# nixorokish/lodestar

Measured on AMD Instinct MI355X. Metric: BLS signature sets verified/sec (1-8 GPUs) + p50 latency @128-set batch, higher is better.
Workload: dtype u32 (381-bit Fp, 12x32-bit Montgomery limbs); 1 GPU; cfg2: 1024 single-pubkey gossip sets per call, batchable requests, random-scalar batch in chunks of 16 requests; each of the 16 contexts submits 22 calls per pass (bls_gpu_verify_many, one device pass, chunks and verdicts per call); sets_per_call=1024, contexts_per_gpu=16, calls_per_pass=22, calls_in_flight_per_gpu=352, parallelism=shard-by-request x1

## Files before the change

__graft_entry__.py:

```python
from __future__ import annotations

import hashlib
import sys
from pathlib import Path

ROOT = Path(__file__).resolve().parent
sys.path.insert(0, str(ROOT))


def build() -> None:
    from lodestar_amd.build import build as build_lib
    from lodestar_amd.build import (build_cpu_baseline, build_deposit_host, build_hostsim, build_napi, build_plan_host,
                                    build_smsum_host)

    build_lib(verbose=True)
    build_napi(verbose=True)
    build_hostsim(verbose=True)
    build_smsum_host(verbose=True)
    build_plan_host(verbose=True)
    build_deposit_host(verbose=True)
    build_cpu_baseline(verbose=True)
    import lodestar_amd
    from lodestar_amd._abi import LIB_PATH

    assert LIB_PATH.exists()


def smoke() -> None:
    from lodestar_amd.native import GpuContext, pack_requests
    from oracle import bls_oracle as O

    with GpuContext(0) as gpu:
        msg = hashlib.sha256(b"lodestar-amd smoke").digest()
        h = gpu.hash_to_g2(msg)[0].tobytes()
        (x0, x1), (y0, y1) = O.hash_to_g2(msg)
        expect = b"".join(v.to_bytes(48, "big") for v in (x1, x0, y1, y0))
        assert h == expect, "hash_to_G2 mismatch against the oracle"

        sks = [O.interop_secret_key(i) for i in range(3)]
        msgs = [hashlib.sha256(b"smoke%d" % i).digest() for i in range(3)]
        sigs = [O.g2_compress(O.sign(s, m)) for s, m in zip(sks, msgs)]
        pks = [O.g1_serialize(O.sk_to_pk(s)) for s in sks]
        sets = list(zip(pks, msgs, sigs))
# ... 10 lines not shown
```

include/lodestar_bls.h:

```cpp
#ifndef LODESTAR_BLS_H
#define LODESTAR_BLS_H

#include <stdint.h>

#ifdef __cplusplus
extern "C" {
#endif

enum {
  BLS_CODE_OK = 0,
  BLS_CODE_BAD_ENCODING = 1,
  BLS_CODE_POINT_NOT_ON_CURVE = 2,
  BLS_CODE_POINT_NOT_IN_GROUP = 3,
  BLS_CODE_PK_IS_INFINITY = 6,
  BLS_CODE_INVALID_SIZE = 8,
  BLS_CODE_ZERO_SIGNATURE = 9,
  BLS_CODE_EMPTY_SET = 10,
  BLS_CODE_EMPTY_AGGREGATE = 11
};

typedef struct bls_batch {
  uint32_t n_sets;
  uint32_t n_reqs;
  const uint32_t* req_set_offsets;
// ... 135 lines not shown
                          uint32_t n_slots, uint32_t* frames_out, uint32_t* flags_out);

int bls_gpu_fpm_bench(bls_gpu_ctx* ctx, uint32_t lanes, uint32_t iters, double* ns_per_fpm, double* fpm_per_s);

int bls_gpu_coop_probe(bls_gpu_ctx* ctx, const char* name, uint32_t blocks, uint32_t reps, double* us_per_step,
                       double* ms_total,
                       uint64_t* step_stamps );

int bls_gpu_kernel_probe(bls_gpu_ctx* ctx, const char* name, uint32_t lanes, uint32_t reps, double* ms);

#define BLS_DEBUG_FORCE_EXACT 1u
#define BLS_DEBUG_NO_MSG_DEDUP 2u
#define BLS_DEBUG_NO_MERGED_CHECK 4u
#define BLS_DEBUG_PACK(n) ((uint32_t)(n) << 8)
#define BLS_DEBUG_PACK_MASK 0x300u
#define BLS_DEBUG_SIGAGG_ON 8u
#define BLS_DEBUG_SIGAGG_OFF 16u
#define BLS_DEBUG_NO_UNITS 32u
#define BLS_DEBUG_MSM 64u
#define BLS_DEBUG_MLF_PL(n) ((uint32_t)(n) << 12)
#define BLS_DEBUG_MLF_PL_MASK 0x7000u
#define BLS_DEBUG_GROUP_TEST 128u
#define BLS_DEBUG_MERGED_EVERY_PASS 0x8000u
int bls_gpu_set_debug_flags(bls_gpu_ctx* ctx, uint32_t flags);

#ifdef __cplusplus
}
#endif

#endif
```

lodestar_amd/_abi.py:

```python
from __future__ import annotations

import ctypes
from pathlib import Path

import os

LIB_PATH = Path(os.environ.get("LODESTAR_BLS_LIB") or Path(__file__).resolve().parent / "_native" / "liblodestar_bls.so")

CODE_OK = 0
CODE_BAD_ENCODING = 1
CODE_POINT_NOT_ON_CURVE = 2
CODE_POINT_NOT_IN_GROUP = 3
CODE_PK_IS_INFINITY = 6
CODE_INVALID_SIZE = 8
CODE_ZERO_SIGNATURE = 9
CODE_EMPTY_SET = 10
CODE_EMPTY_AGGREGATE = 11

ERROR_MESSAGES = {
    CODE_BAD_ENCODING: "BLST_ERROR: BLST_BAD_ENCODING",
    CODE_POINT_NOT_ON_CURVE: "BLST_ERROR: BLST_POINT_NOT_ON_CURVE",
    CODE_POINT_NOT_IN_GROUP: "BLST_ERROR: BLST_POINT_NOT_IN_GROUP",
    CODE_PK_IS_INFINITY: "BLST_ERROR: BLST_PK_IS_INFINITY",
    CODE_INVALID_SIZE: "BLST_ERROR: BLST_INVALID_SIZE",
# ... 39 lines not shown
    "bls_gpu_set_scratch_budget",
    "bls_gpu_request_hw_queues",
)
ERR_ADMISSION = -4
SSZ_ROOT = 0x000 | 32
SSZ_UINT64 = 0x100 | 8
SSZ_CHECKPOINT = 0x200 | 40
SSZ_ATTESTATION_DATA = 0x300 | 128
SSZ_TWO_UINT64 = 0x400 | 16
SSZ_BEACON_BLOCK_HEADER = 0x500 | 112
SSZ_DEPOSIT_MESSAGE = 0x600 | 88
SSZ_FORK_DATA = 0x700 | 36
SSZ_SIGNING_DATA = 0x800 | 64
FIELD_OP_D28 = 0x100
DEBUG_FORCE_EXACT = 1
DEBUG_NO_MSG_DEDUP = 2
DEBUG_NO_MERGED_CHECK = 4
DEBUG_SIGAGG_ON = 8
DEBUG_SIGAGG_OFF = 16
DEBUG_NO_UNITS = 32
DEBUG_MSM = 64
DEBUG_GROUP_TEST = 128
DEBUG_MERGED_EVERY_PASS = 0x8000


def DEBUG_MLF_PL(n: int) -> int:
    return n << 12


def DEBUG_PACK(n: int) -> int:
    return n << 8


class BlsBatch(ctypes.Structure):
    _fields_ = [
        ("n_sets", ctypes.c_uint32),
        ("n_reqs", ctypes.c_uint32),
        ("req_set_offsets", ctypes.c_void_p),
        ("req_batchable", ctypes.c_void_p),
        ("pubkeys", ctypes.c_void_p),
        ("set_pk_offsets", ctypes.c_void_p),
        ("pk_indices", ctypes.c_void_p),
        ("messages", ctypes.c_void_p),
        ("signatures", ctypes.c_void_p),
        ("signature_lens", ctypes.c_void_p),
        ("seed", ctypes.c_void_p),
# ... 163 lines not shown
```

lodestar_amd/build.py:

```python
from __future__ import annotations

import concurrent.futures as cf
import hashlib
import json
import os
import re
import subprocess
import sys
from pathlib import Path

ROOT = Path(__file__).resolve().parent.parent
PKG = ROOT / "lodestar_amd"
CSRC = PKG / "csrc"
OUT_DIR = PKG / "_native"
OBJ_DIR = ROOT / "build" / "obj"
LIB = OUT_DIR / "liblodestar_bls.so"
HIPCC = os.environ.get("HIPCC", "/opt/rocm/bin/hipcc")
ARCH = "gfx950"
FLAGS = ["-O3", "-std=c++17", "-fPIC", f"--offload-arch={ARCH}", "-I", str(ROOT / "include"), "-I", str(CSRC)]


def _headers_digest() -> str:
    h = hashlib.sha256()
    for p in sorted(list(CSRC.rglob("*.hpp")) + list((ROOT / "include").glob("*.h"))):
# ... 211 lines not shown
    if out.exists() and stamp.exists() and stamp.read_text() == key:
        return out
    cmd = ["g++", "-O2", "-std=c++17", *(extra or []), "-I", str(CSRC), "-I", str(ROOT / "include"), "-o", str(out),
           str(src)]
    if verbose:
        print("[build]", " ".join(cmd), flush=True)
    subprocess.run(cmd, check=True)
    stamp.write_text(key)
    return out


def build_smsum_host(verbose: bool = True, out: Path | None = None, extra: list[str] | None = None) -> Path:
    return _build_host_program("smsum_host", (), verbose, out, extra)


def build_plan_host(verbose: bool = True, out: Path | None = None, extra: list[str] | None = None) -> Path:
    return _build_host_program("plan_host", ("plan_exports.hpp",), verbose, out, extra)


def build_deposit_host(verbose: bool = True, out: Path | None = None, extra: list[str] | None = None) -> Path:
    return _build_host_program("deposit_host", (), verbose, out, extra)


def build_cpu_baseline(verbose: bool = True) -> Path:
    out = ROOT / "oracle" / "cpu" / "libbls_cpu.so"
    cmd = ["make", "-s", "-C", str(ROOT / "oracle" / "cpu")]
    if verbose:
        print("[build]", " ".join(cmd), flush=True)
    subprocess.run(cmd, check=True)
    return out


def build_napi(verbose: bool = True) -> Path | None:
    hdr_dir = Path("/usr/include/node")
    if not (hdr_dir / "node_api.h").exists():
        return None
    src = ROOT / "integration" / "napi" / "lodestar_bls_napi.c"
    out = OUT_DIR / "lodestar_bls.node"
    key = hashlib.sha256(src.read_bytes() + (ROOT / "include" / "lodestar_bls.h").read_bytes()).hexdigest()[:16]
    stamp = OUT_DIR / ".napi_stamp"
    if out.exists() and stamp.exists() and stamp.read_text() == key:
        return out
    cmd = ["gcc", "-O2", "-shared", "-fPIC", "-I", str(hdr_dir), "-I", str(ROOT / "include"), str(src),
           "-L", str(OUT_DIR), "-llodestar_bls", "-Wl,-rpath,$ORIGIN", "-o", str(out)]
    if verbose:
        print("[build]", " ".join(cmd), flush=True)
    subprocess.run(cmd, check=True)
    stamp.write_text(key)
    return out


if __name__ == "__main__":
    if len(sys.argv) > 2 and sys.argv[1] == "--variant":
        build(variant=sys.argv[2])
        sys.exit(0)
    build(jobs=int(sys.argv[1]) if len(sys.argv) > 1 else None)
    build_napi()
    build_hostsim()
    build_smsum_host()
    build_plan_host()
    build_deposit_host()
    build_cpu_baseline()
```

lodestar_amd/csrc/bls/curve.hpp:

```cpp
#pragma once

#include "field.hpp"

namespace bls {

BLS_HD Fp f_add(const Fp& a, const Fp& b) { return fp_add(a, b); }
BLS_HD Fp f_sub(const Fp& a, const Fp& b) { return fp_sub(a, b); }
BLS_HD Fp f_mul(const Fp& a, const Fp& b) { return fp_mul(a, b); }
BLS_HD Fp f_sqr(const Fp& a) { return fp_sqr(a); }
BLS_HD Fp f_dbl(const Fp& a) { return fp_dbl(a); }
BLS_HD Fp f_neg(const Fp& a) { return fp_neg(a); }
BLS_HD bool f_is_zero(const Fp& a) { return fp_is_zero(a); }
BLS_HD bool f_eq(const Fp& a, const Fp& b) { return fp_eq(a, b); }
BLS_HD Fp f_inv(const Fp& a) { return fp_inv(a); }
BLS_HD void f_set_zero(Fp& a) { a = fp_zero(); }
BLS_HD void f_set_one(Fp& a) { a = c_one(); }

BLS_HD Fp2 f_add(const Fp2& a, const Fp2& b) { return fp2_add(a, b); }
BLS_HD Fp2 f_sub(const Fp2& a, const Fp2& b) { return fp2_sub(a, b); }
BLS_HD Fp2 f_mul(const Fp2& a, const Fp2& b) { return fp2_mul(a, b); }
BLS_HD Fp2 f_sqr(const Fp2& a) { return fp2_sqr(a); }
BLS_HD Fp2 f_dbl(const Fp2& a) { return fp2_dbl(a); }
BLS_HD Fp2 f_neg(const Fp2& a) { return fp2_neg(a); }
BLS_HD bool f_is_zero(const Fp2& a) { return fp2_is_zero(a); }
// ... 290 lines not shown
  T[2] = p3;
#pragma unroll 1
  for (int j = 1; j < 4; ++j) {
    const Jac<F> e = jac_endo_mu(T[j - 1]);
    T[4 * j - 1] = e;
#pragma unroll 1
    for (int i = 1; i < 4; ++i) T[4 * j + i - 1] = jac_add(e, T[i - 1]);
  }
  Jac<F> acc = jac_infinity<F>();
#pragma unroll 1
  for (int w = 15; w >= 0; --w) {
    acc = jac_dbl(jac_dbl(acc));
    const uint32_t d = ((a >> (2 * w)) & 3u) | (((b >> (2 * w)) & 3u) << 2);
    if (d) acc = jac_add(acc, T[d - 1]);
  }
  return acc;
}

BLS_HD void glv_split(uint64_t r64, uint32_t& a, uint32_t& b) {
  a = (uint32_t)r64;
  b = (uint32_t)(r64 >> 32);
}

enum BlsCode : int32_t {
  BLS_OK = 0,
  BLS_BAD_ENCODING = 1,
  BLS_POINT_NOT_ON_CURVE = 2,
  BLS_POINT_NOT_IN_GROUP = 3,
  BLS_PK_IS_INFINITY = 6,
  BLS_INVALID_SIZE = 8,
  BLS_ZERO_SIGNATURE = 9,
  BLS_EMPTY_SET = 10,
  BLS_EMPTY_AGGREGATE = 11,
};

BLS_HD int32_t g1_deserialize96(const uint8_t* b, G1A& out) {
  out.inf = false;
  if (b[0] & 0x80) return BLS_BAD_ENCODING;
  if (b[0] & 0x40) {
    uint8_t acc = b[0] & 0x3f;
    for (int i = 1; i < 96; ++i) acc |= b[i];
    if (acc) return BLS_BAD_ENCODING;
    out.inf = true;
    out.x = fp_zero();
    out.y = fp_zero();
    return BLS_OK;
// ... 111 lines not shown
```

lodestar_amd/csrc/bls/pipeline.hpp:

```cpp
#pragma once

#include "../../../include/lodestar_bls.h"
#include "hash_to_curve.hpp"
#include "pairing.hpp"
#include "plan_shape.hpp"

namespace bls {

enum : int { CH_HQ = 0, CH_RP = 4, CH_RS = 7, CHAIN_WORDS = 13 };

struct PipeBufs {
  uint32_t n_sets, n_reqs, n_chunks, n_indiv;
  const uint32_t* req_off;
  const uint8_t* pubkeys;
  const uint32_t* set_pk_off;
  const uint32_t* pk_idx;
  const G1A* pk_table;
  uint32_t pk_table_n;
  const uint32_t* agg_sets;
  uint32_t n_agg, agg_min;
  const uint8_t* msgs;
  const uint8_t* sigs;
  const uint32_t* sig_lens;
  const uint32_t* seed;
  const uint32_t* msg_uniq;
  const uint32_t* msg_rep;
  uint32_t n_uniq;
  uint32_t scalar_base;
  uint32_t pack;
  uint32_t mlf_pl;
  uint32_t multi_set_rules;
  uint8_t* pk_inf;
  const uint32_t* chunk_off;
  const uint32_t* chunk_reqs;
  const uint32_t* indiv_reqs;
  const uint32_t* fold_groups;
  uint32_t n_fold;
  uint32_t fold;
  G2A* sig;
  int32_t* sig_status;
  G1J* pk;
// ... 79 lines not shown
  if (b.set_pk_off) {
    uint32_t beg = b.set_pk_off[i], end = b.set_pk_off[i + 1];
    if (b.agg_min && end - beg >= b.agg_min) return;
    if (beg == end) code = BLS_EMPTY_AGGREGATE;
    for (uint32_t k = beg; k < end; ++k) {
      uint32_t idx = b.pk_idx[k];
      if (idx >= b.pk_table_n) {
        code = BLS_BAD_ENCODING;
        break;
      }
      acc = jac_add_aff(acc, b.pk_table[idx]);
    }
  } else {
    G1A a;
    code = g1_deserialize96(b.pubkeys + 96ull * i, a);
    if (code == BLS_OK) acc = jac_from_aff(a);
    else if (b.first_bad_pk) note_min_u32(b.first_bad_pk, i);
  }
  b.pk[i] = acc;
  b.pk_status[i] = code;
  if (b.pk_inf) b.pk_inf[i] = (code == BLS_OK && jac_is_inf(acc)) ? 1 : 0;
}

BLS_HD void stage_sig(const PipeBufs& b, uint32_t i) {
  if (i >= b.n_sets) return;
  G2A s;
  s.inf = true;
  s.x = fp2_zero();
  s.y = fp2_zero();
  int32_t code;
  if (b.sig_lens && b.sig_lens[i] != 96) {
    code = BLS_INVALID_SIZE;
  } else {
    code = g2_decompress96(b.sigs + 96ull * i, s);
    if (code == BLS_OK && !g2_in_subgroup(s)) code = BLS_POINT_NOT_IN_GROUP;
  }
  b.sig[i] = s;
  b.sig_status[i] = code;
}

BLS_HD void stage_h2c(const PipeBufs& b, uint32_t i) {
  if (i >= b.n_sets) return;
  uint32_t w[8];
  msg_words_from_bytes(b.msgs + 32ull * i, w);
  b.H[i] = hash_to_g2(w);
}
// ... 206 lines not shown
```

lodestar_amd/csrc/bls_gpu.hip:

```cpp
#include <hip/hip_runtime.h>
#include <stdarg.h>
#include <stdio.h>
#include <string.h>
#include <sys/random.h>
#include <time.h>
#include <unistd.h>

#include <dlfcn.h>
#include <stdlib.h>
#include <zlib.h>

#include <atomic>
#include <mutex>
#include <string>
#include <vector>

#include "bls/deposit.hpp"
#include "bls/group_decode.hpp"
#include "bls/plan.hpp"
#include "launchers.hpp"

using namespace bls;

struct bls_gpu_ctx {
  int device;
  hipStream_t stream;
  hipEvent_t ev0, ev1;
  hipEvent_t ev[9];
  hipEvent_t ev_wait;
  bool wait_block;
  char err[512];
  G1A* table;
  uint32_t table_n, table_cap;
  uint32_t debug_flags;
  bool last_merged_failed;
  uint32_t* msm_state;
  uint8_t* dev_ws;
  size_t dev_ws_cap;
  uint8_t* host_stage;
  uint8_t* host_stage_dev;
  size_t host_stage_cap;
  uint8_t* host_res;
  uint8_t* host_res_dev;
  size_t host_res_cap;
  uint32_t* first_bad;
  uint32_t first_bad_slot;
  CoopEnv coop;
  void* coop_dev;
  std::vector<std::pair<std::string, CoopProg>>* coop_progs;
  std::vector<uint32_t>* coop_frames;
  std::mutex* mu;
  int admitted;
};

#define CTX_LOCK(ctx) std::lock_guard<std::mutex> ctx_guard_(*(ctx)->mu)

// ... 45 lines not shown
  return 0;
}

int ensure_host(bls_gpu_ctx* ctx, size_t bytes) {
  return ensure_mapped(ctx, bytes, &ctx->host_stage, &ctx->host_stage_dev, &ctx->host_stage_cap);
}

template <class T>
void stage_copy(bls_gpu_ctx* ctx, const T* dev_ptr, const void* src, size_t bytes) {
  if (!src || !bytes) return;
  size_t off = (const uint8_t*)dev_ptr - ctx->host_stage_dev;
  memcpy(ctx->host_stage + off, src, bytes);
}

template <class T>
T* res_host(bls_gpu_ctx* ctx, T* dev_ptr) {
  return (T*)(ctx->host_res + ((uint8_t*)dev_ptr - ctx->host_res_dev));
}

}

extern "C" int bls_gpu_device_count(void);
extern "C" void bls_gpu_close(bls_gpu_ctx* ctx);

namespace {

struct CoopHeader {
  char magic[4];
  uint32_t version, n_consts, n_progs, n_steps;
};
struct CoopProgEntry {
  char name[32];
  uint32_t first, n_steps, frame, n_mul;
};

std::string coop_tables_path() {
  const char* env = getenv("BLS_COOP_TABLES");
  if (env && *env) return env;
  Dl_info info;
  if (dladdr((void*)&bls_gpu_device_count, &info) && info.dli_fname) {
    std::string p(info.dli_fname);
    size_t slash = p.rfind('/');
    return (slash == std::string::npos ? std::string(".") : p.substr(0, slash)) + "/coop_tables.bin.gz";
  }
  return "coop_tables.bin.gz";
}
// ... 257 lines not shown
  {
    std::lock_guard<std::mutex> g(g_adm_mu);
    note_runtime_queues();
    bls_admission a;
    const uint32_t nn = g_adm_normal[device] + (high ? 0u : 1u), nh = g_adm_high[device] + (high ? 1u : 0u);
    if (bls_scratch_plan(nn, nh, 0, &a) != 0) {
      init_fail("BLS_ERR_ADMISSION: a %s-priority context on device %d would map %u normal + %u high-priority "
                "contexts onto %u hardware queues (GPU_MAX_HW_QUEUES=%u), reserving %llu MiB of scratch "
                "(%llu MiB per queue for %s) > the %llu MiB budget ($BLS_SCRATCH_BUDGET_MIB); close a context or "
                "lower the context count",
                high ? "high" : "normal", device, nn, nh, a.queues_in_use, a.hw_queues,
                (unsigned long long)(a.scratch_reserved >> 20), (unsigned long long)(a.scratch_per_queue >> 20),
                BLS_SCRATCH_WORST_KERNEL, (unsigned long long)(a.scratch_budget >> 20));
      return BLS_ERR_ADMISSION;
    }
    if (high) ++g_adm_high[device];
    else ++g_adm_normal[device];
  }
  bls_gpu_ctx* ctx = new bls_gpu_ctx();
  memset(ctx, 0, sizeof(*ctx));
  ctx->mu = new std::mutex();
  ctx->device = device;
  ctx->admitted = high ? 2 : 1;
  auto fail = [&](const char* what, hipError_t e) {
    init_fail("bls_gpu_init: %s: %s", what, hipGetErrorString(e));
    bls_gpu_close(ctx);
    return -1;
  };
  hipError_t e = hipSetDevice(device);
  if (e != hipSuccess) return fail("hipSetDevice", e);
  int prio_lo = 0, prio_hi = 0;
  (void)hipDeviceGetStreamPriorityRange(&prio_lo, &prio_hi);
  if ((e = hipStreamCreateWithPriority(&ctx->stream, hipStreamNonBlocking, high ? prio_hi : prio_lo)) != hipSuccess)
    return fail("hipStreamCreateWithPriority", e);
  if ((e = hipEventCreate(&ctx->ev0)) != hipSuccess || (e = hipEventCreate(&ctx->ev1)) != hipSuccess)
    return fail("hipEventCreate", e);
  for (int i = 0; i < 9; ++i)
    if ((e = hipEventCreate(&ctx->ev[i])) != hipSuccess) return fail("hipEventCreate", e);
  if ((e = hipEventCreateWithFlags(&ctx->ev_wait, hipEventDisableTiming)) != hipSuccess)
    return fail("hipEventCreateWithFlags", e);
  if (load_coop_tables(ctx) != 0) {
    init_fail("bls_gpu_init: %s", ctx->err);
    bls_gpu_close(ctx);
    return -1;
  }
  if ((e = hipMalloc(&ctx->first_bad, 2 * sizeof(uint32_t))) != hipSuccess ||
      (e = hipMemset(ctx->first_bad, 0xFF, 2 * sizeof(uint32_t))) != hipSuccess)
    return fail("first_bad", e);
  if ((e = hipMalloc(&ctx->msm_state, sizeof(uint32_t) * MSM_STATE_WORDS)) != hipSuccess ||
      (e = hipMemset(ctx->msm_state, 0, sizeof(uint32_t) * MSM_STATE_WORDS)) != hipSuccess)
    return fail("msm_state", e);
  *out = ctx;
  return 0;
}

void bls_gpu_close(bls_gpu_ctx* ctx) {
  if (!ctx) return;
  ctx->mu->lock();
  ctx->mu->unlock();
  if (ctx->admitted) {
    std::lock_guard<std::mutex> g(g_adm_mu);
    if (ctx->admitted == 2) --g_adm_high[ctx->device];
    else --g_adm_normal[ctx->device];
    ctx->admitted = 0;
  }
  (void)hipSetDevice(ctx->device);
  if (ctx->stream) (void)hipStreamSynchronize(ctx->stream);
  if (ctx->table) (void)hipFree(ctx->table);
  if (ctx->dev_ws) (void)hipFree(ctx->dev_ws);
  if (ctx->host_stage) (void)hipHostFree(ctx->host_stage);
  if (ctx->host_res) (void)hipHostFree(ctx->host_res);
  if (ctx->first_bad) (void)hipFree(ctx->first_bad);
  if (ctx->msm_state) (void)hipFree(ctx->msm_state);
  if (ctx->ev0) (void)hipEventDestroy(ctx->ev0);
  if (ctx->ev1) (void)hipEventDestroy(ctx->ev1);
  if (ctx->ev_wait) (void)hipEventDestroy(ctx->ev_wait);
  for (int i = 0; i < 9; ++i)
    if (ctx->ev[i]) (void)hipEventDestroy(ctx->ev[i]);
  if (ctx->coop_dev) (void)hipFree(ctx->coop_dev);
  delete ctx->coop_progs;
  delete ctx->coop_frames;
  if (ctx->stream) (void)hipStreamDestroy(ctx->stream);
  delete ctx->mu;
  delete ctx;
}

const char* bls_gpu_last_error(const bls_gpu_ctx* ctx) { return ctx ? ctx->err : "no context"; }

int64_t bls_gpu_load_pubkeys(bls_gpu_ctx* ctx, const uint8_t* pks, uint32_t n, uint32_t pk_len, int32_t* codes) {
  CTX_LOCK(ctx);
  if (pk_len != 48 && pk_len != 96) {
    snprintf(ctx->err, sizeof(ctx->err), "pk_len must be 48 or 96");
    return -1;
  }
  HIPC(ctx, hipSetDevice(ctx->device));
  if (ctx->table_n + n > ctx->table_cap) {
    uint32_t cap = (ctx->table_n + n) + (ctx->table_n + n) / 2 + 1024;
    G1A* t = nullptr;
    HIPC(ctx, hipMalloc(&t, sizeof(G1A) * (size_t)cap));
    if (ctx->table) {
      HIPC(ctx, hipMemcpyAsync(t, ctx->table, sizeof(G1A) * (size_t)ctx->table_n, hipMemcpyDeviceToDevice,
                               ctx->stream));
      HIPC(ctx, hipStreamSynchronize(ctx->stream));
      HIPC(ctx, hipFree(ctx->table));
    }
    ctx->table = t;
    ctx->table_cap = cap;
  }
  if (n == 0) return ctx->table_n;
  size_t in_bytes = (size_t)pk_len * n;
  Carver cv{nullptr, 0};
  cv.take<uint8_t>(in_bytes);
  cv.take<int32_t>(n);
  if (ensure_dev(ctx, cv.off) || ensure_host(ctx, cv.off)) return -1;
  Carver c2{ctx->dev_ws, 0};
  uint8_t* d_in = c2.take<uint8_t>(in_bytes);
  int32_t* d_codes = c2.take<int32_t>(n);
  HIPC(ctx, hipMemcpyAsync(d_in, pks, in_bytes, hipMemcpyHostToDevice, ctx->stream));
  HIPC(ctx, launch_k_load_pubkeys(d_in, n, pk_len, ctx->table + ctx->table_n, d_codes, ctx->stream));
  std::vector<int32_t> host_codes(n);
  HIPC(ctx, hipMemcpyAsync(host_codes.data(), d_codes, sizeof(int32_t) * n, hipMemcpyDeviceToHost, ctx->stream));
  HIPC(ctx, hipStreamSynchronize(ctx->stream));
  if (codes) memcpy(codes, host_codes.data(), sizeof(int32_t) * n);
  for (uint32_t i = 0; i < n; ++i)
    if (host_codes[i] != 0) return ctx->table_n;
  ctx->table_n += n;
  return ctx->table_n;
}

int bls_gpu_validate_pubkeys(bls_gpu_ctx* ctx, const uint8_t* pks, uint32_t n, uint32_t pk_len, int32_t* codes) {
  CTX_LOCK(ctx);
  if ((pk_len != 48 && pk_len != 96) || !codes) {
    snprintf(ctx->err, sizeof(ctx->err), "pk_len must be 48 or 96 and codes non-null");
    return -2;
  }
  if (n == 0) return 0;
  HIPC(ctx, hipSetDevice(ctx->device));
  const size_t in_bytes = (size_t)pk_len * n;
  Carver cv{nullptr, 0};
  cv.take<uint8_t>(in_bytes);
  cv.take<int32_t>(n);
  if (ensure_dev(ctx, cv.off)) return -1;
  Carver c2{ctx->dev_ws, 0};
  uint8_t* d_in = c2.take<uint8_t>(in_bytes);
  int32_t* d_codes = c2.take<int32_t>(n);
  HIPC(ctx, hipMemcpyAsync(d_in, pks, in_bytes, hipMemcpyHostToDevice, ctx->stream));
  HIPC(ctx, launch_k_validate_pubkeys(d_in, n, pk_len, d_codes, ctx->stream));
  HIPC(ctx, hipMemcpyAsync(codes, d_codes, sizeof(int32_t) * n, hipMemcpyDeviceToHost, ctx->stream));
// ... 409 lines not shown
    if (sh.partial || sh.merged) {
      ptree[0] = c.take<Fp12>((sh.n_total + FPROD_FAN - 1) / FPROD_FAN);
      ptree[1] = c.take<Fp12>((sh.n_total + FPROD_FAN - 1) / FPROD_FAN);
    }
  }
  void carve_res(Carver& c) {
    b.chunk_ok = c.take<int32_t>(sh.n_chunks);
    b.indiv_verdict = c.take<int32_t>(sh.R);
    g.verdict = c.take<int32_t>(sh.grp_cap);
    b.req_status_host = c.take<int32_t>(sh.R);
    b.flag_count_host = c.take<uint32_t>(1);
    merged_ok = sh.merged ? c.take<int32_t>(1) : nullptr;
  }

  void fill_fields() {
    b.first_bad_pk = b.pubkeys ? ctx->first_bad + ctx->first_bad_slot : nullptr;
    b.first_bad_pk_next = ctx->first_bad + (ctx->first_bad_slot ^ 1u);
    b.init_set_flag = sh.init_set_flag;
    b.n_sets = sh.n;
    b.n_reqs = sh.R;
    b.n_chunks = sh.n_chunks;
    b.pk_table = ctx->table;
    b.pk_table_n = ctx->table_n;
    b.scalar_base = a.scalar_base;
    b.pack = sh.pack;
    b.mlf_pl = sh.mlf_pl;
    b.multi_set_rules = sh.partial ? 1u : 0u;
    b.sigagg = sh.sigagg ? 1u : 0u;
    b.unit_base = sh.unit_base;
    b.n_units = sh.n_units;
    b.indiv_vbase = sh.indiv_vbase;
    b.n_agg = (uint32_t)pl.agg_list.size();
    b.agg_min = pl.agg_list.empty() ? 0u : BLS_AGG_WAVE_MIN;
    b.n_uniq = sh.dedup ? sh.n_uniq : 0;
  }

  template <class T>
  void stage_vec(const T* dev_ptr, const std::vector<T>& v) {
    stage_copy(ctx, dev_ptr, v.data(), sizeof(T) * v.size());
  }

  void copy_plans() {
    if (sh.use_units) {
      stage_vec(b.set_unit, pl.units.set_unit);
      stage_vec(unit_rep_dev, pl.units.unit_rep);
      stage_vec(b.unit_off, pl.units.unit_off);
// ... 1106 lines not shown
```

lodestar_amd/csrc/kernels/k_chain.hip:

```cpp
#define BLS_FP_D28 1
#define BLS_FP2_PRIM 1
#include "../launchers.hpp"

using namespace bls;

static_assert(BLS_BLOCK == BLS_FP2_SLOT_LANES, "the Fp2 primitive's LDS slot holds one wavefront per block");

namespace {

__device__ __noinline__ void iso_jac_nl(G2J* out, const Fp* q) { *out = iso_map_jac(Fp2{q[0], q[1]}, Fp2{q[2], q[3]}); }

__device__ __noinline__ void g2_mul_aff(G2J* out, const G2A* in, uint64_t k) { *out = aff_mul_u64(*in, k); }
__device__ __noinline__ void g2_mul_r(G2J* out, const G2A* in, uint64_t k, G2J* T) {
  uint32_t a, b;
  glv_split(k, a, b);
  *out = in->inf ? jac_infinity<Fp2>() : jac_mul_glv<Fp2>(jac_from_aff(*in), a, b, T);
}
__device__ __noinline__ void g1_mul_r(G1J* out, const G1J* in, uint64_t k, G1J* T) {
  uint32_t a, b;
  glv_split(k, a, b);
  *out = jac_mul_glv<Fp>(*in, a, b, T);
}
__device__ __noinline__ void g2_add(G2J* out, const G2J* a, const G2J* b) { *out = jac_add(*a, *b); }

__device__ __noinline__ void g2_to_aff(G2A* out, const G2J* in) {
  if (jac_is_inf(*in)) {
    out->x = fp2_zero();
    out->y = fp2_zero();
    out->inf = true;
    return;
  }
  const Fp ni = fp_inv_gcd(fp_add(fp_sqr(in->z.c0), fp_sqr(in->z.c1)));
  const Fp2 zi = Fp2{fp_mul(in->z.c0, ni), fp_neg(fp_mul(in->z.c1, ni))};
  const Fp2 zi2 = fp2_sqr(zi);
  out->x = fp2_mul(in->x, zi2);
  out->y = fp2_mul(in->y, fp2_mul(zi2, zi));
  out->inf = false;
}

__device__ __noinline__ void g2_mul_x_aff(G2J* out, const G2J* p) {
  G2A a;
  g2_to_aff(&a, p);
  g2_mul_aff(out, &a, (uint64_t)BLS_X_ABS);
  out->y = fp2_neg(out->y);
// ... 49 lines not shown

__device__ __noinline__ void chain_role_sub(const G2A* sigs, uint8_t* chain_st, uint32_t i) {
  const G2A sig = sigs[i];
  G2J xs;
  g2_mul_aff(&xs, &sig, (uint64_t)BLS_X_ABS);
  chain_st[4 * i + 1] = jac_eq(g2_psi(jac_from_aff(sig)), jac_neg(xs)) ? 0 : 1;
}

__device__ __noinline__ void chain_role_rs(Fp* chain, const G2A* sigs, const uint32_t* seed, uint32_t scalar_base,
                                           G2J* rtab2, uint32_t i) {
  Fp* o = chain + (size_t)CHAIN_WORDS * i;
  const G2A sig = sigs[i];
  G2J RS;
  g2_mul_r(&RS, &sig, set_scalar(seed, scalar_base + i), rtab2 + 15ull * i);
  o[CH_RS + 0] = RS.x.c0;
  o[CH_RS + 1] = RS.x.c1;
  o[CH_RS + 2] = RS.y.c0;
  o[CH_RS + 3] = RS.y.c1;
  o[CH_RS + 4] = RS.z.c0;
  o[CH_RS + 5] = RS.z.c1;
}

__device__ __noinline__ void chain_role_rp(Fp* chain, const G1J* pks, uint8_t* chain_st, const uint32_t* seed,
                                           uint32_t scalar_base, G1J* rtab1, uint32_t i) {
  Fp* o = chain + (size_t)CHAIN_WORDS * i;
  G1J RP;
  const G1J pk = pks[i];
  g1_mul_r(&RP, &pk, set_scalar(seed, scalar_base + i), rtab1 + 15ull * i);
  chain_st[4 * i + 3] = jac_is_inf(RP) ? 1 : 0;
  if (jac_is_inf(RP)) return;
  o[CH_RP + 0] = RP.x;
  o[CH_RP + 1] = RP.y;
  o[CH_RP + 2] = RP.z;
}

#define BLS_CHAIN_ATTR __attribute__((amdgpu_waves_per_eu(2)))
__global__ __launch_bounds__(BLS_BLOCK) BLS_CHAIN_ATTR void k_chain(PipeBufs b, uint32_t blocks_per_role,
                                                                   uint32_t roles) {
  uint32_t role = 0, nth = blockIdx.x / blocks_per_role;
  for (uint32_t m = roles;; m &= m - 1) {
    if (nth-- == 0) {
      role = (uint32_t)__builtin_ctz(m);
      break;
    }
  }
  const uint32_t i = (blockIdx.x % blocks_per_role) * BLS_BLOCK + threadIdx.x;
  if (i >= b.n_sets) return;
  if (role == 0 ? ((b.msg_rep && b.msg_rep[i] != i) || b.set_flag[i]) : chain_skip(b, i)) return;
  if (role == 0) chain_role_h(b.chain, b.q, b.chain_st, i);
  else if (role == 1) chain_role_sub(b.sig, b.chain_st, i);
  else if (role == 2) chain_role_rs(b.chain, b.sig, b.seed, b.scalar_base, b.rtab2, i);
  else chain_role_rp(b.chain, b.pk, b.chain_st, b.seed, b.scalar_base, b.rtab1, i);
}

__global__ __launch_bounds__(BLS_BLOCK) void k_chain_done(PipeBufs b) {
  BLS_TAIL_PRIO();
  const uint32_t i = blockIdx.x * BLS_BLOCK + threadIdx.x;
  if (i >= b.n_sets) return;
  b.chain_live[i] = 0u;
  if (b.pk_status[i] != BLS_OK || b.sig_status[i] != BLS_OK || jac_is_inf(b.pk[i])) {
    store_one(&b.f[i]);
    return;
  }
  if (b.sig[i].inf || b.set_flag[i]) {
    flag_exact(b, i);
    return;
  }
  const uint8_t* st = b.chain_st + 4 * i;
  if (st[1]) {
    b.sig_status[i] = BLS_POINT_NOT_IN_GROUP;
    store_one(&b.f[i]);
    return;
  }
  const uint32_t rep = b.msg_rep ? b.msg_rep[i] : i;
  if (b.chain_st[4 * rep + 0] || st[3]) {
// ... 22 lines not shown
```

lodestar_amd/csrc/kernels/k_pk.hip:

```cpp
#include "../launchers.hpp"

using namespace bls;

__global__ __launch_bounds__(BLS_BLOCK) void k_pk(PipeBufs b) {
  const uint32_t i = blockIdx.x * BLS_BLOCK + threadIdx.x;
  if (i < b.n_sets) b.set_flag[i] = b.init_set_flag;
  if (i == 0) {
    *b.flag_count = 0u;
    if (b.first_bad_pk_next) *b.first_bad_pk_next = 0xFFFFFFFFu;
  }
  stage_pk(b, i);
}

__global__ __launch_bounds__(BLS_BLOCK) void k_pk_agg(PipeBufs b) {
  __shared__ G1J part[BLS_BLOCK];
  const uint32_t lane = threadIdx.x;
  const uint32_t i = b.agg_sets[blockIdx.x];
  const uint32_t beg = b.set_pk_off[i], end = b.set_pk_off[i + 1];
  G1J acc = jac_infinity<Fp>();
  bool bad = false;
  for (uint32_t k = beg + lane; k < end; k += BLS_BLOCK) {
    const uint32_t idx = b.pk_idx[k];
    if (idx >= b.pk_table_n) bad = true;
    else acc = jac_add_aff(acc, b.pk_table[idx]);
// ... 20 lines not shown
}

__global__ __launch_bounds__(BLS_BLOCK) void k_aggregate(PipeBufs b, uint8_t* out96) {
  uint32_t i = blockIdx.x * BLS_BLOCK + threadIdx.x;
  stage_pk(b, i);
  if (i < b.n_sets) g1_serialize96(jac_to_aff(b.pk[i]), out96 + 96ull * i);
}

__global__ __launch_bounds__(BLS_BLOCK) void k_load_pubkeys(const uint8_t* pks, uint32_t n, uint32_t pk_len,
                                                            G1A* out, int32_t* codes) {
  uint32_t i = blockIdx.x * BLS_BLOCK + threadIdx.x;
  if (i >= n) return;
  G1A a;
  int32_t c = pk_len == 48 ? g1_decompress48(pks + 48ull * i, a) : g1_deserialize96(pks + 96ull * i, a);
  if (c != BLS_OK) {
    a.inf = true;
    a.x = fp_zero();
    a.y = fp_zero();
  }
  out[i] = a;
  codes[i] = c;
}

__global__ __launch_bounds__(BLS_BLOCK) void k_validate_pubkeys(const uint8_t* pks, uint32_t n, uint32_t pk_len,
                                                                int32_t* codes) {
  uint32_t i = blockIdx.x * BLS_BLOCK + threadIdx.x;
  if (i >= n) return;
  G1A a;
  int32_t c = pk_len == 48 ? g1_decompress48(pks + 48ull * i, a) : g1_deserialize96(pks + 96ull * i, a);
  if (c == BLS_OK && a.inf) c = BLS_PK_IS_INFINITY;
  if (c == BLS_OK && !g1_in_subgroup(a)) c = BLS_POINT_NOT_IN_GROUP;
  codes[i] = c;
}

hipError_t launch_k_validate_pubkeys(const uint8_t* pks, uint32_t n, uint32_t pk_len, int32_t* codes, hipStream_t s) {
  k_validate_pubkeys<<<bls_grid_for(n), BLS_BLOCK, 0, s>>>(pks, n, pk_len, codes);
  return hipGetLastError();
}

__global__ __launch_bounds__(BLS_BLOCK) void k_status(PipeBufs b) {
  BLS_TAIL_PRIO();
  const uint32_t r = blockIdx.x * BLS_BLOCK + threadIdx.x;
  stage_req_status(b, r);
  if (b.req_status_host && r < b.n_reqs) b.req_status_host[r] = b.req_status[r];
  if (r == 0 && b.flag_count_host) *b.flag_count_host = b.n_sets ? *b.flag_count : 0u;
}
// ... 19 lines not shown
```

lodestar_amd/csrc/kernels/k_pre.hip:

```cpp
#define BLS_FP_D28 1
#include "../launchers.hpp"

using namespace bls;

__device__ __noinline__ void pre_rpts(const PipeBufs& b, uint32_t j) {
  const uint32_t i = j >> 1, which = j & 1u;
  if (b.pk_status[i] != BLS_OK || jac_is_inf(b.pk[i])) return;
  const G1J p = which == 0 ? b.pk[i] : jac_from_aff(g1_generator());
  uint32_t a, c;
  glv_split(set_scalar(b.seed, b.scalar_base + i), a, c);
  const G1J q = jac_mul_glv<Fp>(p, a, c, b.rtab1 + 15ull * j);
  b.rpts[j] = q;
  if (which == 0 && jac_is_inf(q)) b.set_flag[i] = 1u;
}

__device__ __forceinline__ uint32_t pre_rpts_base(const PipeBufs& b) {
  return (pre_lanes(b) + BLS_BLOCK - 1) / BLS_BLOCK * BLS_BLOCK;
}

#ifndef BLS_PRE_WAVES
#define BLS_PRE_WAVES 3
#endif
__global__ __launch_bounds__(BLS_BLOCK) __attribute__((amdgpu_waves_per_eu(BLS_PRE_WAVES))) void k_pre(PipeBufs b) {
  const uint32_t t = blockIdx.x * BLS_BLOCK + threadIdx.x;
  const uint32_t base = pre_rpts_base(b);
  if (t < base) stage_pre(b, t);
  else if (b.rpts && t < base + 2 * b.n_sets) pre_rpts(b, t - base);
}

__global__ __launch_bounds__(BLS_BLOCK) void k_qdup(PipeBufs b) { stage_qdup(b, blockIdx.x * BLS_BLOCK + threadIdx.x); }

hipError_t launch_k_pre(const PipeBufs& b, hipStream_t s) {
  const uint32_t lanes = (pre_lanes(b) + BLS_BLOCK - 1) / BLS_BLOCK * BLS_BLOCK + (b.rpts ? 2 * b.n_sets : 0u);
  k_pre<<<bls_grid_for(lanes), BLS_BLOCK, 0, s>>>(b);
  hipError_t e = hipGetLastError();
  if (e != hipSuccess || !b.msg_rep) return e;
  k_qdup<<<bls_grid_for(8 * b.n_sets), BLS_BLOCK, 0, s>>>(b);
  return hipGetLastError();
}
```

lodestar_amd/csrc/launchers.hpp:

```cpp
#pragma once

#include <hip/hip_runtime.h>

#include "bls/pipeline.hpp"

#define BLS_BLOCK 64

#define BLS_TAIL_PRIO() __builtin_amdgcn_s_setprio(3)

static inline unsigned bls_grid_for(uint32_t n) { return (n + BLS_BLOCK - 1) / BLS_BLOCK; }

hipError_t launch_k_pk(const bls::PipeBufs& b, hipStream_t s);
hipError_t launch_k_pk_agg(const bls::PipeBufs& b, hipStream_t s);
#define BLS_AGG_WAVE_MIN 16u
hipError_t launch_k_aggregate(const bls::PipeBufs& b, uint8_t* out96, hipStream_t s);
hipError_t launch_k_load_pubkeys(const uint8_t* pks, uint32_t n, uint32_t pk_len, bls::G1A* out, int32_t* codes,
                                 hipStream_t s);
hipError_t launch_k_status(const bls::PipeBufs& b, hipStream_t s);
hipError_t launch_k_validate_pubkeys(const uint8_t* pks, uint32_t n, uint32_t pk_len, int32_t* codes, hipStream_t s);
namespace bls {
struct DepositBufs;
}
hipError_t launch_k_deposit(const bls::PipeBufs& b, const bls::DepositBufs& d, hipStream_t s);
hipError_t launch_k_pre(const bls::PipeBufs& b, hipStream_t s);
hipError_t launch_k_exact(const bls::PipeBufs& b, hipStream_t s);
hipError_t launch_k_chain(const bls::PipeBufs& b, hipStream_t s, uint32_t roles = 0xFu);
struct MsmBufs {
  uint32_t* cnt;
  uint32_t* ticket;
  uint32_t* off;
  uint32_t* seg_off;
  uint32_t* ent;
  uint32_t* sorted;
  bls::G2J* seg_sum;
  bls::G2J* bucket;
  bls::G2J* win;
};
#define MSM_BUCKETS 1020u
size_t msm_seg_cap(uint32_t n_sets);
#define MSM_STATE_WORDS (MSM_BUCKETS + 2u)
// ... 64 lines not shown
```

Before: 4.165 million sets/s.

## Precompute per-pubkey comb tables for G1 random-scalar multiplication

At pubkey load time a kernel builds a 4-teeth comb table of 15 affine points (batch-inverted) for each registered key, plus one for the G1 generator. During verification, single-key sets use a comb multiplication with GLV endomorphism instead of building a runtime window table and running a double-and-add chain. This cuts doublings and per-set table construction for the r*PK and r*G scalar multiplies. In exchange it uses about 1.4 KB of device memory per key and adds build time when keys are loaded.

```diff
diff --git a/__graft_entry__.py b/__graft_entry__.py
--- a/__graft_entry__.py
+++ b/__graft_entry__.py
@@ -10,8 +10,8 @@
 
 def build() -> None:
     from lodestar_amd.build import build as build_lib
-    from lodestar_amd.build import (build_cpu_baseline, build_deposit_host, build_hostsim, build_napi, build_plan_host,
-                                    build_smsum_host)
+    from lodestar_amd.build import (build_comb_host, build_cpu_baseline, build_deposit_host, build_hostsim, build_napi,
+                                    build_plan_host, build_smsum_host)
 
     build_lib(verbose=True)
     build_napi(verbose=True)
@@ -19,6 +19,7 @@
     build_smsum_host(verbose=True)
     build_plan_host(verbose=True)
     build_deposit_host(verbose=True)
+    build_comb_host(verbose=True)
     build_cpu_baseline(verbose=True)
     import lodestar_amd
     from lodestar_amd._abi import LIB_PATH
diff --git a/include/lodestar_bls.h b/include/lodestar_bls.h
--- a/include/lodestar_bls.h
+++ b/include/lodestar_bls.h
@@ -181,6 +181,7 @@
 #define BLS_DEBUG_MLF_PL_MASK 0x7000u
 #define BLS_DEBUG_GROUP_TEST 128u
 #define BLS_DEBUG_MERGED_EVERY_PASS 0x8000u
+#define BLS_DEBUG_NO_PK_COMB 0x10000u
 int bls_gpu_set_debug_flags(bls_gpu_ctx* ctx, uint32_t flags);
 
 #ifdef __cplusplus
diff --git a/lodestar_amd/_abi.py b/lodestar_amd/_abi.py
--- a/lodestar_amd/_abi.py
+++ b/lodestar_amd/_abi.py
@@ -85,6 +85,7 @@
 DEBUG_MSM = 64
 DEBUG_GROUP_TEST = 128
 DEBUG_MERGED_EVERY_PASS = 0x8000
+DEBUG_NO_PK_COMB = 0x10000
 
 
 def DEBUG_MLF_PL(n: int) -> int:
diff --git a/lodestar_amd/build.py b/lodestar_amd/build.py
--- a/lodestar_amd/build.py
+++ b/lodestar_amd/build.py
@@ -257,6 +257,10 @@
     return _build_host_program("deposit_host", (), verbose, out, extra)
 
 
+def build_comb_host(verbose: bool = True, out: Path | None = None, extra: list[str] | None = None) -> Path:
+    return _build_host_program("comb_host", (), verbose, out, extra)
+
+
 def build_cpu_baseline(verbose: bool = True) -> Path:
     out = ROOT / "oracle" / "cpu" / "libbls_cpu.so"
     cmd = ["make", "-s", "-C", str(ROOT / "oracle" / "cpu")]
@@ -295,4 +299,5 @@
     build_smsum_host()
     build_plan_host()
     build_deposit_host()
+    build_comb_host()
     build_cpu_baseline()
diff --git a/lodestar_amd/csrc/bls/curve.hpp b/lodestar_amd/csrc/bls/curve.hpp
--- a/lodestar_amd/csrc/bls/curve.hpp
+++ b/lodestar_amd/csrc/bls/curve.hpp
@@ -336,6 +336,68 @@
   b = (uint32_t)(r64 >> 32);
 }
 
+enum : int { G1_COMB_ROWS = 15, G1_COMB_WORDS = 30 };
+
+BLS_HD uint32_t g1_comb_digit(uint32_t v, int j) {
+  return ((v >> j) & 1u) | (((v >> (8 + j)) & 1u) << 1) | (((v >> (16 + j)) & 1u) << 2) |
+         (((v >> (24 + j)) & 1u) << 3);
+}
+
+BLS_HD G1J g1_comb_mul(const Fp* rows, uint32_t a, uint32_t b) {
+  G1J acc = jac_infinity<Fp>();
+#pragma unroll 1
+  for (int s = 15; s >= 0; --s) {
+    const bool endo = !(s & 1);
+    if (!endo && !jac_is_inf(acc)) acc = jac_dbl(acc);
+    const uint32_t k = g1_comb_digit(endo ? b : a, s >> 1);
+    if (k) {
+      G1A q;
+      q.x = rows[2 * (k - 1)];
+      q.y = rows[2 * (k - 1) + 1];
+      q.inf = false;
+      if (endo) q.x = fp_mul(q.x, c_g1_beta());
+      acc = jac_add_aff(acc, q);
+    }
+  }
+  return acc;
+}
+
+BLS_HD bool g1_comb_build(const G1A& p, G1J* T, Fp* rows) {
+  if (p.inf) return false;
+  G1J t = jac_from_aff(p);
+  T[0] = t;
+#pragma unroll 1
+  for (int w = 1; w < 4; ++w) {
+#pragma unroll 1
+    for (int i = 0; i < 8; ++i) t = jac_dbl(t);
+    T[(1 << w) - 1] = t;
+  }
+#pragma unroll 1
+  for (uint32_t k = 3; k < 16; ++k) {
+    const uint32_t low = k & (0u - k);
+    if (low != k) T[k - 1] = jac_add(T[(k ^ low) - 1], T[low - 1]);
+  }
+  Fp run = T[0].z;
+  rows[0] = run;
+#pragma unroll 1
+  for (int k = 1; k < G1_COMB_ROWS; ++k) {
+    run = fp_mul(run, T[k].z);
+    rows[k] = run;
+  }
+  if (fp_is_zero(run)) return false;
+  Fp inv = fp_inv_gcd(run);
+#pragma unroll 1
+  for (int k = G1_COMB_ROWS - 1; k >= 0; --k) {
+    const G1J e = T[k];
+    const Fp zi = k ? fp_mul(inv, rows[k - 1]) : inv;
+    if (k) inv = fp_mul(inv, e.z);
+    const Fp zi2 = fp_sqr(zi);
+    rows[2 * k] = fp_mul(e.x, zi2);
+    rows[2 * k + 1] = fp_mul(e.y, fp_mul(zi2, zi));
+  }
+  return true;
+}
+
 enum BlsCode : int32_t {
   BLS_OK = 0,
   BLS_BAD_ENCODING = 1,
diff --git a/lodestar_amd/csrc/bls/pipeline.hpp b/lodestar_amd/csrc/bls/pipeline.hpp
--- a/lodestar_amd/csrc/bls/pipeline.hpp
+++ b/lodestar_amd/csrc/bls/pipeline.hpp
@@ -17,6 +17,10 @@
   const uint32_t* pk_idx;
   const G1A* pk_table;
   uint32_t pk_table_n;
+  const Fp* pk_comb;
+  const uint8_t* pk_comb_ok;
+  uint32_t pk_comb_n;
+  const Fp* g1_comb;
   const uint32_t* agg_sets;
   uint32_t n_agg, agg_min;
   const uint8_t* msgs;
@@ -142,6 +146,16 @@
   if (b.pk_inf) b.pk_inf[i] = (code == BLS_OK && jac_is_inf(acc)) ? 1 : 0;
 }
 
+BLS_HD const Fp* set_comb_rows(const uint32_t* set_pk_off, const uint32_t* pk_idx, const Fp* comb,
+                               const uint8_t* comb_ok, uint32_t comb_n, uint32_t i) {
+  if (!comb || !set_pk_off) return nullptr;
+  const uint32_t beg = set_pk_off[i];
+  if (set_pk_off[i + 1] - beg != 1u) return nullptr;
+  const uint32_t idx = pk_idx[beg];
+  if (idx >= comb_n || !comb_ok[idx]) return nullptr;
+  return comb + (size_t)G1_COMB_WORDS * idx;
+}
+
 BLS_HD void stage_sig(const PipeBufs& b, uint32_t i) {
   if (i >= b.n_sets) return;
   G2A s;
diff --git a/lodestar_amd/csrc/bls_gpu.hip b/lodestar_amd/csrc/bls_gpu.hip
--- a/lodestar_amd/csrc/bls_gpu.hip
+++ b/lodestar_amd/csrc/bls_gpu.hip
@@ -32,6 +32,11 @@
   char err[512];
   G1A* table;
   uint32_t table_n, table_cap;
+  Fp* comb;
+  uint8_t* comb_ok;
+  uint32_t comb_cap, comb_n;
+  bool comb_off;
+  Fp* g1_comb;
   uint32_t debug_flags;
   bool last_merged_failed;
   uint32_t* msm_state;
@@ -123,6 +128,8 @@
 
 extern "C" int bls_gpu_device_count(void);
 extern "C" void bls_gpu_close(bls_gpu_ctx* ctx);
+static bool pk_comb_on();
+static void g1_comb_init(bls_gpu_ctx* ctx);
 
 namespace {
 
@@ -426,6 +433,7 @@
   ctx->mu = new std::mutex();
   ctx->device = device;
   ctx->admitted = high ? 2 : 1;
+  ctx->comb_off = !pk_comb_on();
   auto fail = [&](const char* what, hipError_t e) {
     init_fail("bls_gpu_init: %s: %s", what, hipGetErrorString(e));
     bls_gpu_close(ctx);
@@ -454,6 +462,7 @@
   if ((e = hipMalloc(&ctx->msm_state, sizeof(uint32_t) * MSM_STATE_WORDS)) != hipSuccess ||
       (e = hipMemset(ctx->msm_state, 0, sizeof(uint32_t) * MSM_STATE_WORDS)) != hipSuccess)
     return fail("msm_state", e);
+  if (!ctx->comb_off) g1_comb_init(ctx);
   *out = ctx;
   return 0;
 }
@@ -471,6 +480,9 @@
   (void)hipSetDevice(ctx->device);
   if (ctx->stream) (void)hipStreamSynchronize(ctx->stream);
   if (ctx->table) (void)hipFree(ctx->table);
+  if (ctx->comb) (void)hipFree(ctx->comb);
+  if (ctx->comb_ok) (void)hipFree(ctx->comb_ok);
+  if (ctx->g1_comb) (void)hipFree(ctx->g1_comb);
   if (ctx->dev_ws) (void)hipFree(ctx->dev_ws);
   if (ctx->host_stage) (void)hipHostFree(ctx->host_stage);
   if (ctx->host_res) (void)hipHostFree(ctx->host_res);
@@ -491,6 +503,103 @@
 
 const char* bls_gpu_last_error(const bls_gpu_ctx* ctx) { return ctx ? ctx->err : "no context"; }
 
+static bool pk_comb_on() {
+  static const bool on = [] {
+    const char* e = getenv("BLS_PK_COMB");
+    return !(e && *e && atoi(e) == 0);
+  }();
+  return on;
+}
+
+static uint32_t pk_comb_max_keys() {
+  uint64_t mb = 4096;
+  const char* e = getenv("BLS_PK_COMB_MAX_MB");
+  if (e && *e) mb = strtoull(e, nullptr, 10);
+  const uint64_t keys = (mb << 20) / (sizeof(Fp) * G1_COMB_WORDS);
+  return keys > 0xFFFFFFFFull ? 0xFFFFFFFFu : (uint32_t)keys;
+}
+
+static void comb_drop(bls_gpu_ctx* ctx) {
+  (void)hipGetLastError();
+  if (ctx->comb) (void)hipFree(ctx->comb);
+  if (ctx->comb_ok) (void)hipFree(ctx->comb_ok);
+  ctx->comb = nullptr;
+  ctx->comb_ok = nullptr;
+  ctx->comb_cap = ctx->comb_n = 0;
+  ctx->comb_off = true;
+}
+
+static void g1_comb_init(bls_gpu_ctx* ctx) {
+  const size_t off_tmp = 256, off_ok = off_tmp + sizeof(G1J) * G1_COMB_ROWS;
+  static_assert(sizeof(G1A) <= 256, "the key sits before the builder's workspace");
+  uint8_t* buf = nullptr;
+  Fp* rows = nullptr;
+  const G1A g = g1_generator();
+  uint8_t ok = 0;
+  const bool good =
+      hipMalloc(&buf, off_ok + 16) == hipSuccess && hipMalloc(&rows, sizeof(Fp) * G1_COMB_WORDS) == hipSuccess &&
+      hipMemcpy(buf, &g, sizeof(g), hipMemcpyHostToDevice) == hipSuccess &&
+      launch_k_comb_build((const G1A*)buf, 1, (G1J*)(buf + off_tmp), rows, buf + off_ok, ctx->stream) == hipSuccess &&
+      hipStreamSynchronize(ctx->stream) == hipSuccess &&
+      hipMemcpy(&ok, buf + off_ok, 1, hipMemcpyDeviceToHost) == hipSuccess;
+  if (buf) (void)hipFree(buf);
+  if (good && ok) {
+    ctx->g1_comb = rows;
+    return;
+  }
+  (void)hipGetLastError();
+  if (rows) (void)hipFree(rows);
+}
+
+static void comb_grow(bls_gpu_ctx* ctx, uint32_t table_cap) {
+  if (ctx->comb_off) return;
+  const uint32_t max_keys = pk_comb_max_keys();
+  const uint32_t want = table_cap < max_keys ? table_cap : max_keys;
+  if (want <= ctx->comb_cap) return;
+  Fp* rows = nullptr;
+  uint8_t* ok = nullptr;
+  bool good = hipMalloc(&rows, sizeof(Fp) * G1_COMB_WORDS * (size_t)want) == hipSuccess &&
+              hipMalloc(&ok, (size_t)want) == hipSuccess;
+  if (good && ctx->comb_n)
+    good = hipMemcpyAsync(rows, ctx->comb, sizeof(Fp) * G1_COMB_WORDS * (size_t)ctx->comb_n, hipMemcpyDeviceToDevice,
+                          ctx->stream) == hipSuccess &&
+           hipMemcpyAsync(ok, ctx->comb_ok, ctx->comb_n, hipMemcpyDeviceToDevice, ctx->stream) == hipSuccess &&
+           hipStreamSynchronize(ctx->stream) == hipSuccess;
+  if (!good) {
+    if (rows) (void)hipFree(rows);
+    if (ok) (void)hipFree(ok);
+    comb_drop(ctx);
+    return;
+  }
+  if (ctx->comb) (void)hipFree(ctx->comb);
+  if (ctx->comb_ok) (void)hipFree(ctx->comb_ok);
+  ctx->comb = rows;
+  ctx->comb_ok = ok;
+  ctx->comb_cap = want;
+}
+
+static void comb_build_new(bls_gpu_ctx* ctx, uint32_t table_n) {
+  if (ctx->comb_off || !ctx->comb) return;
+  const uint32_t end = table_n < ctx->comb_cap ? table_n : ctx->comb_cap;
+  if (end <= ctx->comb_n) return;
+  const uint32_t BATCH = 1u << 16;
+  const uint32_t todo = end - ctx->comb_n;
+  G1J* tmp = nullptr;
+  bool good = hipMalloc(&tmp, sizeof(G1J) * G1_COMB_ROWS * (size_t)(todo < BATCH ? todo : BATCH)) == hipSuccess;
+  for (uint32_t at = ctx->comb_n; good && at < end; at += BATCH) {
+    const uint32_t m = end - at < BATCH ? end - at : BATCH;
+    good = launch_k_comb_build(ctx->table + at, m, tmp, ctx->comb + (size_t)G1_COMB_WORDS * at, ctx->comb_ok + at,
+                               ctx->stream) == hipSuccess;
+  }
+  good = good && hipStreamSynchronize(ctx->stream) == hipSuccess;
+  if (tmp) (void)hipFree(tmp);
+  if (!good) {
+    comb_drop(ctx);
+    return;
+  }
+  ctx->comb_n = end;
+}
+
 int64_t bls_gpu_load_pubkeys(bls_gpu_ctx* ctx, const uint8_t* pks, uint32_t n, uint32_t pk_len, int32_t* codes) {
   CTX_LOCK(ctx);
   if (pk_len != 48 && pk_len != 96) {
@@ -510,6 +619,7 @@
     }
     ctx->table = t;
     ctx->table_cap = cap;
+    comb_grow(ctx, cap);
   }
   if (n == 0) return ctx->table_n;
   size_t in_bytes = (size_t)pk_len * n;
@@ -528,6 +638,7 @@
   if (codes) memcpy(codes, host_codes.data(), sizeof(int32_t) * n);
   for (uint32_t i = 0; i < n; ++i)
     if (host_codes[i] != 0) return ctx->table_n;
+  comb_build_new(ctx, ctx->table_n + n);
   ctx->table_n += n;
   return ctx->table_n;
 }
@@ -983,6 +1094,12 @@
     b.n_chunks = sh.n_chunks;
     b.pk_table = ctx->table;
     b.pk_table_n = ctx->table_n;
+    if (ctx->comb && !(ctx->debug_flags & BLS_DEBUG_NO_PK_COMB)) {
+      b.pk_comb = ctx->comb;
+      b.pk_comb_ok = ctx->comb_ok;
+      b.pk_comb_n = ctx->comb_n;
+    }
+    if (!(ctx->debug_flags & BLS_DEBUG_NO_PK_COMB)) b.g1_comb = ctx->g1_comb;
     b.scalar_base = a.scalar_base;
     b.pack = sh.pack;
     b.mlf_pl = sh.mlf_pl;
diff --git a/lodestar_amd/csrc/kernels/k_chain.hip b/lodestar_amd/csrc/kernels/k_chain.hip
--- a/lodestar_amd/csrc/kernels/k_chain.hip
+++ b/lodestar_amd/csrc/kernels/k_chain.hip
@@ -20,6 +20,11 @@
   uint32_t a, b;
   glv_split(k, a, b);
   *out = jac_mul_glv<Fp>(*in, a, b, T);
+}
+__device__ __noinline__ void g1_comb_r(G1J* out, const Fp* rows, uint64_t k) {
+  uint32_t a, b;
+  glv_split(k, a, b);
+  *out = g1_comb_mul(rows, a, b);
 }
 __device__ __noinline__ void g2_add(G2J* out, const G2J* a, const G2J* b) { *out = jac_add(*a, *b); }
 
@@ -115,11 +120,19 @@
 }
 
 __device__ __noinline__ void chain_role_rp(Fp* chain, const G1J* pks, uint8_t* chain_st, const uint32_t* seed,
-                                           uint32_t scalar_base, G1J* rtab1, uint32_t i) {
+                                           uint32_t scalar_base, G1J* rtab1, const uint32_t* set_pk_off,
+                                           const uint32_t* pk_idx, const Fp* comb, const uint8_t* comb_ok,
+                                           uint32_t comb_n, uint32_t i) {
   Fp* o = chain + (size_t)CHAIN_WORDS * i;
   G1J RP;
-  const G1J pk = pks[i];
-  g1_mul_r(&RP, &pk, set_scalar(seed, scalar_base + i), rtab1 + 15ull * i);
+  const uint64_t r = set_scalar(seed, scalar_base + i);
+  const Fp* rows = set_comb_rows(set_pk_off, pk_idx, comb, comb_ok, comb_n, i);
+  if (rows) {
+    g1_comb_r(&RP, rows, r);
+  } else {
+    const G1J pk = pks[i];
+    g1_mul_r(&RP, &pk, r, rtab1 + 15ull * i);
+  }
   chain_st[4 * i + 3] = jac_is_inf(RP) ? 1 : 0;
   if (jac_is_inf(RP)) return;
   o[CH_RP + 0] = RP.x;
@@ -143,7 +156,8 @@
   if (role == 0) chain_role_h(b.chain, b.q, b.chain_st, i);
   else if (role == 1) chain_role_sub(b.sig, b.chain_st, i);
   else if (role == 2) chain_role_rs(b.chain, b.sig, b.seed, b.scalar_base, b.rtab2, i);
-  else chain_role_rp(b.chain, b.pk, b.chain_st, b.seed, b.scalar_base, b.rtab1, i);
+  else chain_role_rp(b.chain, b.pk, b.chain_st, b.seed, b.scalar_base, b.rtab1, b.set_pk_off, b.pk_idx, b.pk_comb,
+                     b.pk_comb_ok, b.pk_comb_n, i);
 }
 
 __global__ __launch_bounds__(BLS_BLOCK) void k_chain_done(PipeBufs b) {
diff --git a/lodestar_amd/csrc/kernels/k_pk.hip b/lodestar_amd/csrc/kernels/k_pk.hip
--- a/lodestar_amd/csrc/kernels/k_pk.hip
+++ b/lodestar_amd/csrc/kernels/k_pk.hip
@@ -66,6 +66,20 @@
   codes[i] = c;
 }
 
+__global__ __launch_bounds__(BLS_BLOCK) __attribute__((amdgpu_waves_per_eu(1, 2))) void k_comb_build(
+    const G1A* keys, uint32_t n, G1J* tmp, Fp* rows, uint8_t* ok) {
+  const uint32_t i = blockIdx.x * BLS_BLOCK + threadIdx.x;
+  if (i >= n) return;
+  const G1A p = keys[i];
+  ok[i] = g1_comb_build(p, tmp + (size_t)G1_COMB_ROWS * i, rows + (size_t)G1_COMB_WORDS * i) ? 1 : 0;
+}
+
+hipError_t launch_k_comb_build(const G1A* keys, uint32_t n, G1J* tmp, Fp* rows, uint8_t* ok, hipStream_t s) {
+  if (n == 0) return hipSuccess;
+  k_comb_build<<<bls_grid_for(n), BLS_BLOCK, 0, s>>>(keys, n, tmp, rows, ok);
+  return hipGetLastError();
+}
+
 __global__ __launch_bounds__(BLS_BLOCK) void k_validate_pubkeys(const uint8_t* pks, uint32_t n, uint32_t pk_len,
                                                                 int32_t* codes) {
   uint32_t i = blockIdx.x * BLS_BLOCK + threadIdx.x;
diff --git a/lodestar_amd/csrc/kernels/k_pre.hip b/lodestar_amd/csrc/kernels/k_pre.hip
--- a/lodestar_amd/csrc/kernels/k_pre.hip
+++ b/lodestar_amd/csrc/kernels/k_pre.hip
@@ -3,15 +3,22 @@
 
 using namespace bls;
 
-__device__ __noinline__ void pre_rpts(const PipeBufs& b, uint32_t j) {
+__device__ __noinline__ void pre_rpts(const int32_t* pk_status, const G1J* pk, const uint32_t* seed,
+                                      uint32_t scalar_base, G1J* rtab1, G1J* rpts, uint32_t* set_flag,
+                                      const Fp* rows, uint32_t j) {
   const uint32_t i = j >> 1, which = j & 1u;
-  if (b.pk_status[i] != BLS_OK || jac_is_inf(b.pk[i])) return;
-  const G1J p = which == 0 ? b.pk[i] : jac_from_aff(g1_generator());
+  if (pk_status[i] != BLS_OK || jac_is_inf(pk[i])) return;
   uint32_t a, c;
-  glv_split(set_scalar(b.seed, b.scalar_base + i), a, c);
-  const G1J q = jac_mul_glv<Fp>(p, a, c, b.rtab1 + 15ull * j);
-  b.rpts[j] = q;
-  if (which == 0 && jac_is_inf(q)) b.set_flag[i] = 1u;
+  glv_split(set_scalar(seed, scalar_base + i), a, c);
+  G1J q;
+  if (rows) {
+    q = g1_comb_mul(rows, a, c);
+  } else {
+    const G1J p = which == 0 ? pk[i] : jac_from_aff(g1_generator());
+    q = jac_mul_glv<Fp>(p, a, c, rtab1 + 15ull * j);
+  }
+  rpts[j] = q;
+  if (which == 0 && jac_is_inf(q)) set_flag[i] = 1u;
 }
 
 __device__ __forceinline__ uint32_t pre_rpts_base(const PipeBufs& b) {
@@ -25,7 +32,12 @@
   const uint32_t t = blockIdx.x * BLS_BLOCK + threadIdx.x;
   const uint32_t base = pre_rpts_base(b);
   if (t < base) stage_pre(b, t);
-  else if (b.rpts && t < base + 2 * b.n_sets) pre_rpts(b, t - base);
+  else if (b.rpts && t < base + 2 * b.n_sets) {
+    const uint32_t j = t - base;
+    const Fp* rows = (j & 1u) ? b.g1_comb
+                              : set_comb_rows(b.set_pk_off, b.pk_idx, b.pk_comb, b.pk_comb_ok, b.pk_comb_n, j >> 1);
+    pre_rpts(b.pk_status, b.pk, b.seed, b.scalar_base, b.rtab1, b.rpts, b.set_flag, rows, j);
+  }
 }
 
 __global__ __launch_bounds__(BLS_BLOCK) void k_qdup(PipeBufs b) { stage_qdup(b, blockIdx.x * BLS_BLOCK + threadIdx.x); }
diff --git a/lodestar_amd/csrc/launchers.hpp b/lodestar_amd/csrc/launchers.hpp
--- a/lodestar_amd/csrc/launchers.hpp
+++ b/lodestar_amd/csrc/launchers.hpp
@@ -16,6 +16,8 @@
 hipError_t launch_k_aggregate(const bls::PipeBufs& b, uint8_t* out96, hipStream_t s);
 hipError_t launch_k_load_pubkeys(const uint8_t* pks, uint32_t n, uint32_t pk_len, bls::G1A* out, int32_t* codes,
                                  hipStream_t s);
+hipError_t launch_k_comb_build(const bls::G1A* keys, uint32_t n, bls::G1J* tmp, bls::Fp* rows, uint8_t* ok,
+                               hipStream_t s);
 hipError_t launch_k_status(const bls::PipeBufs& b, hipStream_t s);
 hipError_t launch_k_validate_pubkeys(const uint8_t* pks, uint32_t n, uint32_t pk_len, int32_t* codes, hipStream_t s);
 namespace bls {
```

After: 4.301 million sets/s (median of 6 runs). 3.3% higher.
